# MILVLG/mmnas

Measured on AMD Instinct MI355X. Metric: supernet fwd+bwd steps/sec (VQA arch, bs=64), higher is better.
Workload: dtype f32 (bf16x6 split-operand MFMA, fp32 accumulate); 1 GPU; Net_Search supernet WEIGHT step: sample + fwd + BCE(sum) + bwd (+ gradient all-reduce), HSIZE 256, B=64/GPU, 100x2048 regions + 14 tokens, dropout 0.1 (search_vqa.py:279-292; BASELINE configs[2]); global_batch=64, parallelism=dp1, grad_allreduce=none, rccl_ranks=1, rank_id_sum_ok=True, lstm_fallback=False, dp_rows=1, dp_buckets=3, optimizer_in_step=False, gemm_split=6, hip_force_dev_kernarg=1

## Files before the change

### mmnas_amd/csrc/common.h

```cpp
#pragma once
#include <hip/hip_runtime.h>
#include <hip/hip_ext.h>
#include <stdint.h>
#include <stdio.h>
#include "../../include/mmnas_hip.h"
#include "rng.h"
#include "switches.h"

namespace mmnas {

typedef float f32x4 __attribute__((ext_vector_type(4)));
typedef float f32x16 __attribute__((ext_vector_type(16)));

void set_error(const char* fmt, ...);
int check_launch(const char* what);

#define MMNAS_REQUIRE(cond, code, ...) \
  do { if (!(cond)) { ::mmnas::set_error(__VA_ARGS__); return (code); } } while (0)

template <int CTRL, int ROW_MASK>
__device__ __forceinline__ float dpp_move(float old, float src) {
  return __int_as_float(__builtin_amdgcn_update_dpp(__float_as_int(old), __float_as_int(src), CTRL, ROW_MASK, 0xf, false));
}
__device__ __forceinline__ float wave_sum(float v) {
// ... 58 lines not shown

bool glimpse1_supported(int MID);
int glimpse1_fwd(const float* h0, const float* w0, const float* b0, float* l0, long rows0, const float* h1, const float* w1,
                 const float* b1, float* l1, long rows1, int MID, hipStream_t st);
struct NodeLnBwd {
  float* dz; float* dt;
  float* part;
  DropCfg drop;
};
int node_mix_bwd_impl(const float* const* z, const float* const* ln_a, const float* const* ln_b, int n, const float* gate,
                      const float* dout, float* d_active, int active, float* dgate, float* ws, int M, int d, float eps,
                      hipStream_t stream, bool reduce, int* nwg_out, const NodeLnBwd* lnb = nullptr);
int mixed_reduce_many(const float* const* parts, float* const* dgates, const int* nwg, const int* n, int count, hipStream_t st);
int mha_core_fwd_pair(const mmnas_mha_desc* d0, const mmnas_mha_desc* d1, hipStream_t st);
int mha_core_fwd_indexed(const mmnas_mha_desc* d, const int* kv_idx, hipStream_t st);
int transpose2d(const float* in, float* out, int R, int C, hipStream_t st);
int glimpse1_bwd_blocks(long rows, int MID);
int glimpse1_bwd(const float* dlog, const float* h, const float* w2, float gate_scale, int gated, float* dh, float* db1, float* dW2,
                 float* part, long rows, int MID, hipStream_t st, AuxReduce* aux);

int attflat_pool_fwd_packed(const float* logits, const float* x, float* probs, float* pooled, int B, int S, int d, int G, const int* off, hipStream_t st);
int attflat_pool_bwd_packed(const float* probs, const float* x, const float* dpooled, float* dlogits, float* dx, int B, int S, int d, int G,
                            const int* off, hipStream_t st);

constexpr int ADD_MANY_MAX = 24;
int add_many(const float* const* srcs, int n, float* y, size_t count, hipStream_t st);

static inline int cdiv(long a, long b) { return (int)((a + b - 1) / b); }

}
```

### mmnas_amd/csrc/head.hip

```cpp
#include "common.h"

namespace mmnas {

__global__ void __launch_bounds__(256) row_is_zero_kernel(const float* __restrict__ f, uint8_t* __restrict__ mask,
                                                          long rows, int d) {
  const int lane = threadIdx.x & 63;
  const long row = (long)blockIdx.x * 4 + (threadIdx.x >> 6);
  if (row >= rows) return;
  const float* fr = f + row * d;
  bool nz = false;
  if ((d & 3) == 0 && (((uintptr_t)fr) & 15) == 0) {
    for (int c = lane * 4; c < d; c += 256) {
      const float4 v = *reinterpret_cast<const float4*>(fr + c);
      nz |= !(v.x == 0.f && v.y == 0.f && v.z == 0.f && v.w == 0.f);
    }
  } else {
    for (int c = lane; c < d; c += 64) nz |= !(fr[c] == 0.f);
  }
  const unsigned long long any = __ballot(nz);
  if (lane == 0) mask[row] = any ? 0 : 1;
}

constexpr int AF_MAXS = 1024;

constexpr int AF_THREADS = 1024, AF_WAVES = AF_THREADS / 64;

__device__ __forceinline__ float block_reduce(float v, float* red, bool is_max) {
  const int lane = threadIdx.x & 63, w = threadIdx.x >> 6;
  v = is_max ? wave_max(v) : wave_sum(v);
  __syncthreads();
  if (lane == 0) red[w] = v;
  __syncthreads();
  float r = red[0];
  for (int i = 1; i < AF_WAVES; ++i) r = is_max ? fmaxf(r, red[i]) : r + red[i];
  return r;
}

__global__ void __launch_bounds__(AF_THREADS) attflat_pool_fwd_kernel(const float* __restrict__ logits, const float* __restrict__ x,
                                                                      const uint8_t* __restrict__ mask, float* __restrict__ probs,
                                                                      float* __restrict__ pooled, int S, int d, int G,
                                                                      const int* __restrict__ off) {
  __shared__ float sp[AF_MAXS];
  __shared__ float red[AF_WAVES];
  __shared__ float part[AF_WAVES / 4][1024];
  const int b = blockIdx.x, g = blockIdx.y, tid = threadIdx.x;
  const size_t row0 = off ? (size_t)off[b] : (size_t)b * S;
  if (off) S = off[b + 1] - off[b];
  const float* lg = logits + row0 * G + g;
  float m = -INFINITY;
  for (int s = tid; s < S; s += AF_THREADS) {
    float v = lg[(size_t)s * G];
    if (mask && !off && mask[(size_t)b * S + s]) v = -1e9f;
    sp[s] = v;
    m = fmaxf(m, v);
  }
  m = block_reduce(m, red, true);
  float sum = 0.f;
  for (int s = tid; s < S; s += AF_THREADS) {
    const float e = expf(sp[s] - m);
    sp[s] = e;
// ... 15 lines not shown
      int s = rg;
      for (; s + 12 < S; s += 16) {
        a0 += sp[s] * xb[(size_t)s * d + j];
        a1 += sp[s + 4] * xb[(size_t)(s + 4) * d + j];
        a2 += sp[s + 8] * xb[(size_t)(s + 8) * d + j];
        a3 += sp[s + 12] * xb[(size_t)(s + 12) * d + j];
      }
      for (; s < S; s += 4) a0 += sp[s] * xb[(size_t)s * d + j];
      part[rg][j - j0] = (a0 + a1) + (a2 + a3);
    }
    __syncthreads();
    for (int j = j0 + tid; j < min(d, j0 + 1024); j += AF_THREADS)
      pooled[(size_t)b * G * d + (size_t)g * d + j] = (part[0][j - j0] + part[1][j - j0]) + (part[2][j - j0] + part[3][j - j0]);
    __syncthreads();
  }
}

__global__ void __launch_bounds__(AF_THREADS) attflat_pool_bwd_kernel(const float* __restrict__ probs, const float* __restrict__ x,
                                                                      const uint8_t* __restrict__ mask,
                                                                      const float* __restrict__ dpooled, float* __restrict__ dlogits,
                                                                      float* __restrict__ dx, int S, int d, int G,
                                                                      const int* __restrict__ off) {
  __shared__ float st[AF_MAXS];
  __shared__ float red[AF_WAVES];
  const int b = blockIdx.x, tid = threadIdx.x, lane = tid & 63, w = tid >> 6;
  const size_t row0 = off ? (size_t)off[b] : (size_t)b * S;
  if (off) S = off[b + 1] - off[b];
  const float* xb = x + row0 * d;
  for (int g = 0; g < G; ++g) {
    const float* dp = dpooled + (size_t)b * G * d + (size_t)g * d;
// ... 75 lines not shown
      sw.x += dl[i] * hv[i].x; sw.y += dl[i] * hv[i].y; sw.z += dl[i] * hv[i].z; sw.w += dl[i] * hv[i].w;
    }
    *reinterpret_cast<float4*>(&red[0][slot * MID + 4 * c4]) = sb;
    *reinterpret_cast<float4*>(&red[1][slot * MID + 4 * c4]) = sw;
  }
  __syncthreads();
  float* mine = part + (size_t)blockIdx.x * 3 * MID;
  for (int i = threadIdx.x; i < 2 * MID; i += 256) {
    const int a = i < MID ? 0 : 1, c = i - a * MID;
    float v = 0.f;
    for (int q = 0; q < rs; ++q) v += red[a][q * MID + c];
    mine[a * MID + c] = v;
  }
}

__global__ void __launch_bounds__(256) transpose_kernel(const float* __restrict__ in, float* __restrict__ out, int R, int C) {
  __shared__ float t[32][33];
  const int c0 = blockIdx.x * 32, r0 = blockIdx.y * 32, tx = threadIdx.x & 31, ty = threadIdx.x >> 5;
  for (int i = ty; i < 32; i += 8)
    if (r0 + i < R && c0 + tx < C) t[i][tx] = in[(size_t)(r0 + i) * C + c0 + tx];
  __syncthreads();
  for (int i = ty; i < 32; i += 8)
    if (c0 + i < C && r0 + tx < R) out[(size_t)(c0 + i) * R + r0 + tx] = t[tx][i];
}
int transpose2d(const float* in, float* out, int R, int C, hipStream_t st) {
  MMNAS_REQUIRE(in && out && R > 0 && C > 0, MMNAS_E_ARG, "transpose2d: bad arguments");
  ProfScope ps(MMNAS_K_ROWOPS, 0.0, 8.0 * R * C, st);
  MMNAS_LAUNCH(transpose_kernel, dim3((C + 31) / 32, (R + 31) / 32), dim3(256), 0, st, in, out, R, C);
  return check_launch("transpose2d");
}

bool glimpse1_supported(int MID) { return MID >= 4 && MID % 4 == 0 && MID <= 1024; }

int glimpse1_fwd(const float* h0, const float* w0, const float* b0, float* l0, long rows0, const float* h1, const float* w1,
                 const float* b1, float* l1, long rows1, int MID, hipStream_t st) {
  MMNAS_REQUIRE(glimpse1_supported(MID) && h0 && w0 && l0 && rows0 > 0 && (rows1 == 0 || (h1 && w1 && l1)), MMNAS_E_ARG,
                "glimpse1_fwd: bad arguments");
  const Glimpse1Side s0{h0, w0, b0, l0, rows0}, s1{h1, w1, b1, l1, rows1};
  ProfScope ps(MMNAS_K_ROWOPS, 2.0 * (rows0 + rows1) * MID, 4.0 * (rows0 + rows1) * MID, st);
  MMNAS_LAUNCH(glimpse1_fwd_kernel, dim3((unsigned)((rows0 + rows1 + 3) / 4)), dim3(256), 0, st, s0, s1, MID);
  return check_launch("glimpse1_fwd");
}

// ... 41 lines not shown
}

extern "C" int mmnas_attflat_pool_fwd(const float* logits, const float* x, const uint8_t* mask, float* probs,
                                      float* pooled, int B, int S, int d, int G, void* stream) {
  MMNAS_REQUIRE(logits && x && probs && pooled, MMNAS_E_ARG, "attflat_pool_fwd: null pointer");
  MMNAS_REQUIRE(B > 0 && S > 0 && S <= AF_MAXS && d > 0 && G > 0, MMNAS_E_SHAPE, "attflat_pool_fwd: B=%d S=%d d=%d G=%d (S <= %d)",
                B, S, d, G, AF_MAXS);
  MMNAS_LAUNCH(attflat_pool_fwd_kernel, dim3(B, G), dim3(AF_THREADS), 0, (hipStream_t)stream, logits, x, mask, probs, pooled, S, d, G, (const int*)nullptr);
  return check_launch("attflat_pool_fwd");
}
namespace mmnas {
int attflat_pool_fwd_packed(const float* logits, const float* x, float* probs, float* pooled, int B, int S, int d, int G, const int* off, hipStream_t st) {
  MMNAS_REQUIRE(logits && x && probs && pooled && off, MMNAS_E_ARG, "attflat_pool_fwd: null pointer");
  MMNAS_REQUIRE(B > 0 && S > 0 && S <= AF_MAXS && d > 0 && G > 0, MMNAS_E_SHAPE, "attflat_pool_fwd: B=%d S=%d d=%d G=%d (S <= %d)", B, S, d, G, AF_MAXS);
  MMNAS_LAUNCH(attflat_pool_fwd_kernel, dim3(B, G), dim3(AF_THREADS), 0, st, logits, x, (const uint8_t*)nullptr, probs, pooled, S, d, G, off);
  return check_launch("attflat_pool_fwd");
}
int attflat_pool_bwd_packed(const float* probs, const float* x, const float* dpooled, float* dlogits, float* dx, int B, int S, int d, int G,
                            const int* off, hipStream_t st) {
  MMNAS_REQUIRE(probs && x && dpooled && dlogits && dx && off, MMNAS_E_ARG, "attflat_pool_bwd: null pointer");
  MMNAS_REQUIRE(B > 0 && S > 0 && S <= AF_MAXS && d > 0 && G > 0, MMNAS_E_SHAPE, "attflat_pool_bwd: B=%d S=%d d=%d G=%d (S <= %d)", B, S, d, G, AF_MAXS);
  MMNAS_LAUNCH(attflat_pool_bwd_kernel, dim3(B), dim3(AF_THREADS), 0, st, probs, x, (const uint8_t*)nullptr, dpooled, dlogits, dx, S, d, G, off);
  return check_launch("attflat_pool_bwd");
}
}

extern "C" int mmnas_attflat_pool_bwd(const float* probs, const float* x, const uint8_t* mask, const float* dpooled,
                                      float* dlogits, float* dx, int B, int S, int d, int G, void* stream) {
  MMNAS_REQUIRE(probs && x && dpooled && dlogits && dx, MMNAS_E_ARG, "attflat_pool_bwd: null pointer");
  MMNAS_REQUIRE(B > 0 && S > 0 && S <= AF_MAXS && d > 0 && G > 0, MMNAS_E_SHAPE, "attflat_pool_bwd: B=%d S=%d d=%d G=%d (S <= %d)",
// ... 235 lines not shown
```

### mmnas_amd/csrc/ops.hip

```cpp
#include <string.h>
#include <functional>
#include <vector>
#include "common.h"

namespace mmnas {

static inline size_t al(size_t n) { return (n + 255) & ~(size_t)255; }
template <class Op> static inline bool drops(const Op* op) { return (op->flags & MMNAS_F_TRAIN) && op->drop_p > 0.f; }

struct Carver {
  char* base; size_t off;
  explicit Carver(void* p) : base((char*)p), off(0) {}
  float* take(size_t nfloats) { float* r = (float*)(base + off); off += al(nfloats * sizeof(float)); return r; }
};

static void gemm_init(mmnas_gemm_desc& g, int layout, int N, int K, int lda, int ldb, int ldc) {
  memset(&g, 0, sizeof(g));
  g.layout = layout; g.ngroups = 1; g.nseg = 1; g.N = N; g.K = K; g.lda = lda; g.ldb = ldb; g.ldc = ldc;
  g.alpha = 1.f; g.gate_scale = 1.f; g.split_k = 1;
}

struct AttLayout {
  size_t Mq, Mk;
  float *Q, *K, *V, *att, *stats, *z, *biasT;
// ... 1429 lines not shown
    const size_t M = sd.off ? (size_t)sd.M : B * sd.S;
    HeadSideLayout& s = L.s[k];
    s.h = c.take(M * hd->MID); s.logit = c.take(M * hd->G); s.probs = c.take(M * hd->G); s.pooled = c.take(B * hd->G * hd->d);
    s.dpooled = c.take(B * hd->G * hd->d); s.dlog = c.take(M * hd->G); s.dh = c.take(M * hd->MID); s.dxpool = c.take(M * hd->d);
    s.g1part = (hd->G == 1 && glimpse1_supported(hd->MID)) ? c.take((size_t)glimpse1_bwd_blocks((long)M, hd->MID) * 3 * hd->MID) : nullptr;
  }
  L.xo = c.take(B * hd->OUT); L.sum = c.take(B * hd->OUT); L.xy = c.take(B * hd->OUT);
  L.dxy = c.take(B * hd->OUT); L.dsum = c.take(B * hd->OUT);
  L.lnws = c.take(mmnas_layernorm_bwd_ws_floats(hd->B, hd->OUT));
  L.g1proj = (hd->ANS == 1 && glimpse1_supported(hd->OUT)) ? c.take((size_t)glimpse1_bwd_blocks((long)B, hd->OUT) * 3 * hd->OUT) : nullptr;
  L.dlogT = (hd->ANS % 4 != 0 && hd->B % 4 == 0 && hd->ANS > 1) ? c.take((size_t)hd->ANS * B) : nullptr;
  L.total = c.off;
  return L;
}

static int head_check(const mmnas_head* hd, const char* who) {
  MMNAS_REQUIRE(hd, MMNAS_E_ARG, "%s: null descriptor", who);
  MMNAS_REQUIRE(hd->B > 0 && hd->d > 0 && hd->MID > 0 && hd->G > 0 && hd->OUT > 0 && hd->ANS > 0 && hd->sx.S > 0 && hd->sy.S > 0,
                MMNAS_E_SHAPE, "%s: B=%d d=%d MID=%d G=%d OUT=%d ANS=%d Sx=%d Sy=%d", who, hd->B, hd->d, hd->MID, hd->G, hd->OUT,
                hd->ANS, hd->sx.S, hd->sy.S);
  MMNAS_REQUIRE(hd->d % 4 == 0 && hd->MID % 4 == 0 && hd->OUT % 4 == 0, MMNAS_E_SHAPE, "%s: d, MID, OUT must be multiples of 4", who);
  for (int k = 0; k < 2; ++k) {
    const mmnas_attflat_side& sd = k ? hd->sy : hd->sx;
    if (sd.off) MMNAS_REQUIRE(sd.M > 0 && sd.M <= hd->B * sd.S, MMNAS_E_ARG, "%s: packed side %d: M=%d of B*S=%d rows", who, k, sd.M, hd->B * sd.S);
  }
  return MMNAS_OK;
}

}

// ... 42 lines not shown
  }
  const bool g1 = G == 1 && !oc && glimpse1_supported(MID) && head_glimpse1_on();
  if (g1) {
    if ((rc = glimpse1_fwd(L.s[0].h, hd->sx.W2, hd->sx.b2, L.s[0].logit, (long)head_rows(hd, hd->sx), L.s[1].h, hd->sy.W2, hd->sy.b2,
                           L.s[1].logit, (long)head_rows(hd, hd->sy), MID, st)))
      return rc;
  }
  gemm_init(g, MMNAS_GEMM_NT, G, MID, MID, MID, G);
  for (int k = 0; k < 2 && !g1; ++k) {
    const mmnas_attflat_side& sd = *sides[k];
    mmnas_gemm_group& gg = g.g[oc ? 0 : k];
    gg.M = head_rows(hd, sd); gg.A[0] = L.s[k].h; gg.B[0] = sd.W2; gg.bias = sd.b2; gg.C = L.s[k].logit;
    if (oc && (rc = mmnas_gemm(&g, side_stream(k)))) return rc;
  }
  if (!oc && !g1) { g.ngroups = 2; if ((rc = mmnas_gemm(&g, stream))) return rc; }
  for (int k = 0; k < 2; ++k) {
    const mmnas_attflat_side& sd = *sides[k];
    const HeadSideLayout& s = L.s[k];
    void* const ks = side_stream(k);
    if ((rc = sd.off ? attflat_pool_fwd_packed(s.logit, sd.x, s.probs, s.pooled, B, sd.S, d, G, sd.off, (hipStream_t)ks)
                     : mmnas_attflat_pool_fwd(s.logit, sd.x, sd.mask, s.probs, s.pooled, B, sd.S, d, G, ks))) return rc;
    gemm_init(g, MMNAS_GEMM_NT, OUT, G * d, G * d, G * d, OUT);
    g.g[0].M = B; g.g[0].A[0] = s.pooled; g.g[0].B[0] = sd.Wm; g.g[0].bias = sd.bm; g.g[0].C = k ? L.sum : L.xo;
    if (k) { g.g[0].residual = L.xo; g.ldres = OUT; }
    if (k && oc && (rc = ev_fork(oc->enc, st, oc->ovl[1]))) return rc;
    if ((rc = mmnas_gemm(&g, ks))) return rc;
  }
  if ((rc = mmnas_layernorm_fwd(L.sum, hd->ln_a, hd->ln_b, L.xy, B, OUT, hd->eps, stream))) return rc;
  if (L.g1proj && head_glimpse1_on())
    return glimpse1_fwd(L.xy, hd->Wp, hd->bp, hd->logits, B, nullptr, nullptr, nullptr, nullptr, 0, OUT, st);
  gemm_init(g, MMNAS_GEMM_NT, hd->ANS, OUT, OUT, OUT, hd->ANS);
  g.g[0].M = B; g.g[0].A[0] = L.xy; g.g[0].B[0] = hd->Wp; g.g[0].bias = hd->bp; g.g[0].C = hd->logits;
  return mmnas_gemm(&g, stream);
}

extern "C" int mmnas_head_bwd(const mmnas_head* hd, void* stream) {
  int rc = head_check(hd, "head_bwd");
  if (rc) return rc;
  MMNAS_REQUIRE(hd->arena && hd->dlogits && hd->ln_a && hd->dln_a && hd->dln_b && hd->Wp && hd->dWp, MMNAS_E_ARG, "head_bwd: null pointer");
  HeadLayout L = head_layout(hd);
  const bool drop = drops(hd);
  const float gate_scale = drop ? 1.0f / (1.0f - hd->drop_p) : 1.0f;
  const int B = hd->B, d = hd->d, MID = hd->MID, G = hd->G, OUT = hd->OUT, ANS = hd->ANS;
  hipStream_t st = (hipStream_t)stream;
  mmnas_gemm_desc g, w;
  if (L.g1proj && head_glimpse1_on()) {
    AuxReduce pr;
    if ((rc = glimpse1_bwd(hd->dlogits, L.xy, hd->Wp, 1.0f, 0, L.dxy, nullptr, hd->dWp, L.g1proj, B, OUT, st, &pr))) return rc;
    if ((rc = launch_aux_reduce(pr, st))) return rc;
  } else if (L.dlogT && head_projT_on()) {
    if ((rc = transpose2d(hd->dlogits, L.dlogT, B, ANS, st))) return rc;
    gemm_init(g, MMNAS_GEMM_TN, OUT, ANS, B, OUT, OUT);
    g.g[0].M = B; g.g[0].A[0] = L.dlogT; g.g[0].B[0] = hd->Wp; g.g[0].C = L.dxy;
    if ((rc = mmnas_gemm(&g, stream))) return rc;
    gemm_init(w, MMNAS_GEMM_NN, OUT, B, B, OUT, OUT);
    w.g[0].M = ANS; w.g[0].A[0] = L.dlogT; w.g[0].B[0] = L.xy; w.g[0].C = hd->dWp; w.accumulate = 1;
    if ((rc = mmnas_gemm(&w, stream))) return rc;
  } else {
    gemm_init(w, MMNAS_GEMM_TN, OUT, B, ANS, OUT, OUT);
    w.g[0].M = ANS; w.g[0].A[0] = hd->dlogits; w.g[0].B[0] = L.xy; w.g[0].C = hd->dWp; w.accumulate = 1;
    gemm_init(g, MMNAS_GEMM_NN, OUT, ANS, ANS, OUT, OUT);
    g.g[0].M = B; g.g[0].A[0] = hd->dlogits; g.g[0].B[0] = hd->Wp; g.g[0].C = L.dxy;
    if ((rc = mmnas_gemm_pair(&g, &w, stream))) return rc;
  }
  if (hd->dbp && (rc = mmnas_colsum(hd->dlogits, hd->dbp, B, ANS, ANS, stream))) return rc;
  AuxReduce lnred;
  lnred.part = nullptr;
  if ((rc = layernorm_bwd_deferred(L.sum, hd->ln_a, L.dxy, L.dsum, hd->dln_a, hd->dln_b, nullptr, nullptr, L.lnws, 0.f, 0, 0, B, OUT,
                                   hd->eps, st, &lnred)))
    return rc;
  SideCtx* oc = head_overlap_on() ? side_ctx(st, true) : nullptr;
  if (oc && (rc = ev_fork(st, oc->enc, oc->ovl[2]))) return rc;
  for (int k = 1; k >= 0; --k) {
    const mmnas_attflat_side& sd = k ? hd->sy : hd->sx;
    const HeadSideLayout& s = L.s[k];
    MMNAS_REQUIRE(sd.x && sd.dx && sd.dW1 && sd.dW2 && sd.dWm, MMNAS_E_ARG, "head_bwd: side %d null pointer", k);
    hipStream_t st = (oc && k == 0) ? oc->enc : (hipStream_t)stream;
    void* const stream = (void*)st;
    const int M = head_rows(hd, sd);
    gemm_init(w, MMNAS_GEMM_TN, G * d, B, OUT, G * d, G * d);
    w.g[0].M = OUT; w.g[0].A[0] = L.dsum; w.g[0].B[0] = s.pooled; w.g[0].C = sd.dWm; w.accumulate = 1;
    gemm_init(g, MMNAS_GEMM_NN, G * d, OUT, OUT, G * d, G * d);
    g.g[0].M = B; g.g[0].A[0] = L.dsum; g.g[0].B[0] = sd.Wm; g.g[0].C = s.dpooled;
    if ((rc = gemm_pair_aux(&g, &w, k ? &lnred : nullptr, st))) return rc;
    if (sd.dbm && (rc = mmnas_colsum(L.dsum, sd.dbm, B, OUT, OUT, stream))) return rc;
    if ((rc = sd.off ? attflat_pool_bwd_packed(s.probs, sd.x, s.dpooled, s.dlog, s.dxpool, B, sd.S, d, G, sd.off, st)
                     : mmnas_attflat_pool_bwd(s.probs, sd.x, sd.mask, s.dpooled, s.dlog, s.dxpool, B, sd.S, d, G, stream))) return rc;
    AuxReduce g1red;
    g1red.part = nullptr;
    if (G == 1 && glimpse1_supported(MID) && head_glimpse1_on()) {
      if ((rc = glimpse1_bwd(s.dlog, s.h, sd.W2, gate_scale, 1, s.dh, sd.db1, sd.dW2, s.g1part, M, MID, st, &g1red))) return rc;
      if (sd.db2 && (rc = mmnas_colsum(s.dlog, sd.db2, M, G, G, stream))) return rc;
    } else {
    gemm_init(w, MMNAS_GEMM_TN, MID, M, G, MID, MID);
    w.g[0].M = G; w.g[0].A[0] = s.dlog; w.g[0].B[0] = s.h; w.g[0].C = sd.dW2; w.accumulate = 1;
    gemm_init(g, MMNAS_GEMM_NN, MID, G, G, MID, MID);
    g.g[0].M = M; g.g[0].A[0] = s.dlog; g.g[0].B[0] = sd.W2; g.g[0].C = s.dh;
    g.g[0].gate = s.h; g.ldgate = MID; g.gate_scale = gate_scale;
    g.g[0].colsum = sd.db1;
    if ((rc = mmnas_gemm_pair(&g, &w, stream))) return rc;
    if (sd.db2 && (rc = mmnas_colsum(s.dlog, sd.db2, M, G, G, stream))) return rc;
    }
    gemm_init(w, MMNAS_GEMM_TN, d, M, MID, d, d);
    w.g[0].M = MID; w.g[0].A[0] = s.dh; w.g[0].B[0] = sd.x; w.g[0].C = sd.dW1; w.accumulate = 1;
    gemm_init(g, MMNAS_GEMM_NN, d, MID, MID, d, d);
    g.g[0].M = M; g.g[0].A[0] = s.dh; g.g[0].B[0] = sd.W1; g.g[0].C = sd.dx;
    g.g[0].residual = s.dxpool; g.ldres = d;
    if ((rc = gemm_pair_aux(&g, &w, g1red.part ? &g1red : nullptr, st))) return rc;
  }
  if (oc && (rc = ev_fork(oc->enc, st, oc->ovl[3]))) return rc;
  return MMNAS_OK;
}
```

### mmnas_amd/csrc/switches.h

```cpp
#pragma once

namespace mmnas {

int env_int(const char* name, int dflt);

enum SwKind { sw_int, sw_bool, sw_exact1, sw_presence, sw_string };
enum SwPolicy { sw_once, sw_every_call, sw_reload };

struct Switch {
  const char* name;
  int dflt;
  SwKind kind;
  SwPolicy policy;
  const char* help;
  int value;
  int state;

  int get() { return state ? value : read(); }
  int read();
  int reload();
  int set(int v);
  int peek(int* source) const;
};

#define MMNAS_SWITCHES(X) \
   \
  X(chain_overlap, "MMNAS_CHAIN_OVERLAP", 0, bool, once, "language stream beside the leading image-stream operators (mmnas_set_chain_overlap); measured: no gain, DESIGN.md section 5") \
  X(head_overlap, "MMNAS_HEAD_OVERLAP", 0, bool, once, "the answer head's two AttFlat sides on two streams") \
  X(head_glimpse1, "MMNAS_HEAD_GLIMPSE1", 1, bool, every_call, "0: the head's one-glimpse logit layer as GEMM launches (A/B, tests); ops.py reads it too") \
  X(head_projt, "MMNAS_HEAD_PROJT", 1, bool, every_call, "0: the answer projection's gradients from the untransposed loss gradient") \
  X(rel_hoist, "MMNAS_REL_HOIST", 1, bool, once, "relation bias of all lazy-handle operators of a stream in one launch per direction (mmnas_set_rel_hoist); 0: one fused launch per operator (supernet step 4.54 -> 5.00 ms)") \
  X(rel_overlap, "MMNAS_REL_OVERLAP", 0, bool, once, "the image stream's relation launches on a second stream (mmnas_set_rel_overlap); measured slower, +2.5 % on the supernet step") \
  X(node_lnb, "MMNAS_NODE_LNB", 1, bool, once, "architecture step: the sampled candidate's LayerNorm backward inside the node's mix kernel (7.81 -> 7.72 ms, profiles/r06_node_lnb_ab.txt); 0: its own launch") \
  X(guided_hoist, "MMNAS_GUIDED_HOIST", 1, bool, once, "key / value projections of a chain's guided operators as grouped launches (mmnas_set_guided_hoist)") \
  X(rel_fwd_valu, "MMNAS_REL_FWD_VALU", 0, exact1, every_call, "1: a lone RelSelfAtt computes its bias with the per-operator fused kernel instead of the one-operator multi kernel (A/B)") \
  X(side_prio, "MMNAS_SIDE_PRIO", 1, bool, every_call, "0: the chains' extra streams without stream priorities (read when a stream pair is created)") \
  X(side_flush, "MMNAS_SIDE_FLUSH", 0, string, once, "op: side-stream parameter-gradient work released behind every operator instead of once per phase") \
  X(wgrad_live, "MMNAS_WGRAD_LIVE", 1, int, once, "image-stream weight gradients of a padded batch's chain reduce over the 32-row K-tiles that cover the live gradient rows only (mmnas_set_wgrad_live); 0: all B Sy rows") \
   \
  X(small_ops, "MMNAS_SMALL_OPS", 1, bool, once, "SelfAtt of <= 16 rows as one launch forward (mmnas_set_small_ops); 0: the general path") \
  X(small_bwd, "MMNAS_SMALL_BWD", 1, bool, once, "the same operators' backward as two launches (mmnas_set_small_bwd)") \
  X(small_ffn, "MMNAS_SMALL_FFN", 0, int, once, "FeedForward forward as one launch (mmnas_set_small_ffn): 1 four slices of 256 hidden units, 2 eight of 128; measured neutral (profiles/r05_small_ffn_ab.txt)") \
   \
  X(gemm_ln, "MMNAS_GEMM_LN", 0, exact1, once, "1: the merge / last FFN product and its LayerNorm as one row-panel launch (mmnas_set_gemm_ln); measured neutral, profiles/r06_ab.txt") \
// ... 46 lines not shown
```

### mmnas_amd/switches.py

```python
import contextlib
import os

_PARSE = {
    'not0': lambda v: v != '0',
    'is1': lambda v: v == '1',
    'presence': lambda v: v is not None,
    'tri': lambda v: int(v) if v in ('0', '1') else None,
    'side': lambda v: 2 if v == 'rel' else int(v == '1'),
    'string': lambda v: v,
}


class Flag:
    __slots__ = ('name', 'default', 'kind', 'policy', 'help', '_parse', '_state', '_value')

    def __init__(self, name, default, kind, policy, help):
        self.name, self.default, self.kind, self.policy, self.help = name, default, kind, policy, help
        self._parse = _PARSE[kind]
        self._state = None
        self._value = None

    def get(self):
        if self._state is not None:
            return self._value
# ... 27 lines not shown
AUTOGRAD_CHAIN = _flag('MMNAS_AUTOGRAD_CHAIN', False, 'is1', 'every_call', '1: the chain as one autograd node whose inputs are the parameters (stock DDP); measured neutral')
UNPAD = _flag('MMNAS_UNPAD', False, 'is1', 'once', '1: the decoder stream on the valid region rows only (ops.set_unpad): same logits and gradients, supernet step 4.73 -> 3.78 ms (DESIGN.md)')
VGD_HEAD = _flag('MMNAS_VGD_HEAD', False, 'is1', 'once', '1: the grounding head as one native call per direction (ops.set_vgd_head); measurement: README, the grounding head section')
LSTM = _flag('MMNAS_LSTM', True, 'not0', 'every_call', '0: nn.LSTM (MIOpen, ~110 launches per step) instead of the persistent-kernel LSTM')
CONV_IM2COL = _flag('MMNAS_CONV_IM2COL', None, 'tri', 'every_call', 'dense Conv1d: 1 always through the window buffer, 0 direct whenever the shape allows, unset: direct unless the padded grid costs > 25 % more rows')
HEAD_GLIMPSE1 = _flag('MMNAS_HEAD_GLIMPSE1', True, 'not0', 'every_call', '0: one-unit linear layers as GEMM launches (A/B, tests); the native head reads it too')
GEMM_GENERIC = _flag('MMNAS_GEMM_GENERIC', False, 'presence', 'every_call', 'set (to anything): dense Conv1d through the window buffer, as the guarded-load GEMM path needs; gemm.hip reads it too')
ZERO_TERMS = _flag('MMNAS_ZERO_TERMS', True, 'not0', 'every_call', "0: plain parameters instead of the zero-term bookkeeping of the reference's literal lines (zeroterm.py)")
LAZY_REL = _flag('MMNAS_LAZY_REL', True, 'not0', 'import', '0: materialise the relation embeddings as the reference does (read when model/nets.py is imported)')
DP_ROWS = _flag('MMNAS_DP_ROWS', True, 'not0', 'every_call', '0: the embedding gradient exchanged dense instead of by rows (A/B)')
DP_INLINE = _flag('MMNAS_DP_INLINE', True, 'not0', 'every_call', '0: async_op=True + work.wait() instead of collectives issued inline on the communication stream')
DP_TAIL_MAIN = _flag('MMNAS_DP_TAIL_MAIN', True, 'not0', 'import', '0: the end of a data-parallel step on the communication stream, one scatter per bucket (1: -0.7 % on search_vqa_dp1; read when dp.py is imported)')
DP_EARLY_SCATTER = _flag('MMNAS_DP_EARLY_SCATTER', False, 'is1', 'every_call', "1: scatter a bucket's averaged gradients back as soon as its all-reduce is done")
LIB_PATH = _flag('MMNAS_LIB_PATH', None, 'string', 'doc', 'path of the shared library to load instead of mmnas_amd/lib/libmmnas_hip.so (tuning builds; read when _lib.py is imported)')
_flag('MMNAS_REFERENCE_ROOT', None, 'string', 'doc', "a checkout of the reference whose mmnas/ package is merged behind this repository's (mmnas/__init__.py)")
_flag('MMNAS_PROF_DUMP', None, 'string', 'doc', 'file the native profiler appends one row per bracketed launch to (csrc/util.hip)')
_flag('MMNAS_LN_ROWS_STATS', None, 'string', 'doc', 'file tests/test_ln_rows_gpu.py writes the worst LayerNorm error per (kernel, row class, output) to (tests/ln_rows.py)')


@contextlib.contextmanager
def gemm_schedule(rows):
    from . import _lib as L
    known = native()
    for name in rows:
        if name not in known:
            raise ValueError('gemm_schedule: %s is not a row of the native switch table' % name)
    saved = {}
    try:
        for name, v in rows.items():
            saved[name] = os.environ.get(name)
# ... 36 lines not shown
```

Baseline: 244.1 steps/s.

## Fuse answer-head AttFlat sides into shared pool-forward and pool+glimpse backward kernels

Adds a two-side pooling forward kernel and a single backward kernel that does the pooling backward and the one-glimpse logit backward for both AttFlat sides in one launch. It also folds the projection bias column sum into the transpose kernel. The aim is to cut launch count and the intermediate dlog/h round trips in the answer head. The transpose-with-colsum kernel now uses one block per column strip with a serial loop over rows, which lowers parallelism, and a new switch gates the fused path (on by default).

Result: no change. 245.6 steps/s (median of 6 runs) (+0.6%).

```diff
diff --git a/mmnas_amd/csrc/common.h b/mmnas_amd/csrc/common.h
--- a/mmnas_amd/csrc/common.h
+++ b/mmnas_amd/csrc/common.h
@@ -96,7 +96,7 @@
 int mixed_reduce_many(const float* const* parts, float* const* dgates, const int* nwg, const int* n, int count, hipStream_t st);
 int mha_core_fwd_pair(const mmnas_mha_desc* d0, const mmnas_mha_desc* d1, hipStream_t st);
 int mha_core_fwd_indexed(const mmnas_mha_desc* d, const int* kv_idx, hipStream_t st);
-int transpose2d(const float* in, float* out, int R, int C, hipStream_t st);
+int transpose2d(const float* in, float* out, int R, int C, hipStream_t st, float* colsum = nullptr);
 int glimpse1_bwd_blocks(long rows, int MID);
 int glimpse1_bwd(const float* dlog, const float* h, const float* w2, float gate_scale, int gated, float* dh, float* db1, float* dW2,
                  float* part, long rows, int MID, hipStream_t st, AuxReduce* aux);
@@ -105,6 +105,19 @@
 int attflat_pool_bwd_packed(const float* probs, const float* x, const float* dpooled, float* dlogits, float* dx, int B, int S, int d, int G,
                             const int* off, hipStream_t st);
 
+struct HeadBwdSide {
+  const float *probs, *x, *dpooled, *h, *w2;
+  const uint8_t* mask;
+  const int* off;
+  float *dlog, *dxpool, *dh, *part;
+  int S;
+};
+int attflat_pool_fwd_sides(const float* const* logits, const float* const* x, const uint8_t* const* mask, float* const* probs,
+                           float* const* pooled, const int* const* off, const int* S, int B, int d, int G, hipStream_t st);
+bool head_sides_bwd_fits(long rows, int B, int MID);
+int head_sides_bwd(const HeadBwdSide* sides, float* const* db1, float* const* dW2, int B, int d, int MID,
+                   float gate_scale, hipStream_t st, AuxReduce* aux);
+
 constexpr int ADD_MANY_MAX = 24;
 int add_many(const float* const* srcs, int n, float* y, size_t count, hipStream_t st);
 
diff --git a/mmnas_amd/csrc/head.hip b/mmnas_amd/csrc/head.hip
--- a/mmnas_amd/csrc/head.hip
+++ b/mmnas_amd/csrc/head.hip
@@ -36,14 +36,14 @@
   return r;
 }
 
-__global__ void __launch_bounds__(AF_THREADS) attflat_pool_fwd_kernel(const float* __restrict__ logits, const float* __restrict__ x,
-                                                                      const uint8_t* __restrict__ mask, float* __restrict__ probs,
-                                                                      float* __restrict__ pooled, int S, int d, int G,
-                                                                      const int* __restrict__ off) {
+__device__ __forceinline__ void attflat_pool_fwd_body(const float* __restrict__ logits, const float* __restrict__ x,
+                                                      const uint8_t* __restrict__ mask, float* __restrict__ probs,
+                                                      float* __restrict__ pooled, int S, int d, int G,
+                                                      const int* __restrict__ off, const int b, const int g) {
   __shared__ float sp[AF_MAXS];
   __shared__ float red[AF_WAVES];
   __shared__ float part[AF_WAVES / 4][1024];
-  const int b = blockIdx.x, g = blockIdx.y, tid = threadIdx.x;
+  const int tid = threadIdx.x;
   const size_t row0 = off ? (size_t)off[b] : (size_t)b * S;
   if (off) S = off[b + 1] - off[b];
   const float* lg = logits + row0 * G + g;
@@ -89,6 +89,20 @@
       pooled[(size_t)b * G * d + (size_t)g * d + j] = (part[0][j - j0] + part[1][j - j0]) + (part[2][j - j0] + part[3][j - j0]);
     __syncthreads();
   }
+}
+
+__global__ void __launch_bounds__(AF_THREADS) attflat_pool_fwd_kernel(const float* __restrict__ logits, const float* __restrict__ x,
+                                                                      const uint8_t* __restrict__ mask, float* __restrict__ probs,
+                                                                      float* __restrict__ pooled, int S, int d, int G,
+                                                                      const int* __restrict__ off) {
+  attflat_pool_fwd_body(logits, x, mask, probs, pooled, S, d, G, off, blockIdx.x, blockIdx.y);
+}
+
+struct PoolFwdSide { const float* logits; const float* x; const uint8_t* mask; float* probs; float* pooled; const int* off; int S; };
+
+__global__ void __launch_bounds__(AF_THREADS) attflat_pool_fwd2_kernel(const PoolFwdSide s0, const PoolFwdSide s1, int d, int G) {
+  const PoolFwdSide& s = blockIdx.z ? s1 : s0;
+  attflat_pool_fwd_body(s.logits, s.x, s.mask, s.probs, s.pooled, s.S, d, G, s.off, blockIdx.x, blockIdx.y);
 }
 
 __global__ void __launch_bounds__(AF_THREADS) attflat_pool_bwd_kernel(const float* __restrict__ probs, const float* __restrict__ x,
@@ -194,6 +208,136 @@
   }
 }
 
+constexpr int HF_ITER = 4;
+constexpr int HF_CS = 4096;
+
+__device__ __forceinline__ void hf_load(float4 (&hv)[HF_ITER], const float* __restrict__ hb, int r0, int rs, int S, int MID, int c4) {
+#pragma unroll
+  for (int i = 0; i < HF_ITER; ++i) {
+    const int r = r0 + i * rs;
+    hv[i] = r < S ? *reinterpret_cast<const float4*>(hb + (size_t)r * MID + 4 * c4) : make_float4(0.f, 0.f, 0.f, 0.f);
+  }
+}
+
+__global__ void __launch_bounds__(AF_THREADS) head_side_bwd_kernel(const HeadBwdSide s0, const HeadBwdSide s1, int d, int MID,
+                                                                   float gate_scale) {
+  __shared__ float st[AF_MAXS], sp[AF_MAXS], sdl[AF_MAXS];
+  __shared__ float red[AF_WAVES];
+  __shared__ __attribute__((aligned(16))) float cs[2][HF_CS];
+  const HeadBwdSide& sd = blockIdx.y ? s1 : s0;
+  const int b = blockIdx.x, tid = threadIdx.x, lane = tid & 63, w = tid >> 6;
+  int S = sd.S;
+  const size_t row0 = sd.off ? (size_t)sd.off[b] : (size_t)b * S;
+  if (sd.off) S = sd.off[b + 1] - sd.off[b];
+  const float* __restrict__ xb = sd.x + row0 * d;
+  const float* __restrict__ dp = sd.dpooled + (size_t)b * d;
+  const float* __restrict__ hb = sd.h + row0 * MID;
+  const int nc4 = MID >> 2;
+  const int rs = AF_THREADS / nc4;
+  const int c4 = tid % nc4, slot = tid / nc4;
+  const bool colthr = slot < rs;
+  float4 hv[HF_ITER];
+  if (colthr) hf_load(hv, hb, slot, rs, S, MID, c4);
+  for (int s = w; s < S; s += 2 * AF_WAVES) {
+    const int sb = s + AF_WAVES;
+    float a = 0.f, a2 = 0.f;
+    if (sb < S) {
+      for (int j = lane; j < d; j += 64) {
+        a += xb[(size_t)s * d + j] * dp[j];
+        a2 += xb[(size_t)sb * d + j] * dp[j];
+      }
+      a2 = wave_sum(a2);
+      if (lane == 0) st[sb] = a2;
+    } else {
+      for (int j = lane; j < d; j += 64) a += xb[(size_t)s * d + j] * dp[j];
+    }
+    a = wave_sum(a);
+    if (lane == 0) st[s] = a;
+  }
+  __syncthreads();
+  float dot = 0.f;
+  for (int s = tid; s < S; s += AF_THREADS) {
+    const float pr = sd.probs[row0 + s];
+    sp[s] = pr;
+    dot += pr * st[s];
+  }
+  dot = block_reduce(dot, red, false);
+  for (int s = tid; s < S; s += AF_THREADS) {
+    const float pr = sp[s];
+    const bool masked = sd.mask && !sd.off && sd.mask[(size_t)b * S + s];
+    const float dl = masked ? 0.f : pr * (st[s] - dot);
+    sd.dlog[row0 + s] = dl;
+    sdl[s] = dl;
+  }
+  __syncthreads();
+  float* __restrict__ mine = sd.part + (size_t)b * 3 * MID;
+  if (colthr) {
+    const float4 wv = *reinterpret_cast<const float4*>(sd.w2 + 4 * c4);
+    float* __restrict__ dhb = sd.dh + row0 * MID;
+    float4 sb = make_float4(0.f, 0.f, 0.f, 0.f), sw = sb;
+    for (int r0 = slot; r0 < S; r0 += rs * HF_ITER) {
+      float4 hn[HF_ITER];
+      hf_load(hn, hb, r0 + rs * HF_ITER, rs, S, MID, c4);
+#pragma unroll
+      for (int i = 0; i < HF_ITER; ++i) {
+        const int r = r0 + i * rs;
+        if (r < S) {
+          const float dl = sdl[r];
+          float4 o;
+          o.x = hv[i].x > 0.f ? dl * wv.x * gate_scale : 0.f; o.y = hv[i].y > 0.f ? dl * wv.y * gate_scale : 0.f;
+          o.z = hv[i].z > 0.f ? dl * wv.z * gate_scale : 0.f; o.w = hv[i].w > 0.f ? dl * wv.w * gate_scale : 0.f;
+          *reinterpret_cast<float4*>(dhb + (size_t)r * MID + 4 * c4) = o;
+          sb.x += o.x; sb.y += o.y; sb.z += o.z; sb.w += o.w;
+          sw.x += dl * hv[i].x; sw.y += dl * hv[i].y; sw.z += dl * hv[i].z; sw.w += dl * hv[i].w;
+        }
+      }
+#pragma unroll
+      for (int i = 0; i < HF_ITER; ++i) hv[i] = hn[i];
+    }
+    *reinterpret_cast<float4*>(&cs[0][slot * MID + 4 * c4]) = sb;
+    *reinterpret_cast<float4*>(&cs[1][slot * MID + 4 * c4]) = sw;
+  }
+  float* __restrict__ dxb = sd.dxpool + row0 * d;
+  for (int s = w; s < S; s += AF_WAVES) {
+    const float pr = sp[s];
+    for (int j = 4 * lane; j < d; j += 256) {
+      const float4 dv = *reinterpret_cast<const float4*>(dp + j);
+      float4 o = make_float4(0.f, 0.f, 0.f, 0.f);
+      o.x += pr * dv.x; o.y += pr * dv.y; o.z += pr * dv.z; o.w += pr * dv.w;
+      *reinterpret_cast<float4*>(dxb + (size_t)s * d + j) = o;
+    }
+  }
+  __syncthreads();
+  for (int i = tid; i < 2 * MID; i += AF_THREADS) {
+    const int a = i < MID ? 0 : 1, c = i - a * MID;
+    float v = 0.f;
+    for (int q = 0; q < rs; ++q) v += cs[a][q * MID + c];
+    mine[a * MID + c] = v;
+  }
+}
+
+bool head_sides_bwd_fits(long rows, int B, int MID) { return glimpse1_supported(MID) && glimpse1_bwd_blocks(rows, MID) >= B; }
+
+int head_sides_bwd(const HeadBwdSide* sides, float* const* db1, float* const* dW2, int B, int d, int MID,
+                   float gate_scale, hipStream_t st, AuxReduce* aux) {
+  MMNAS_REQUIRE(sides && aux && B > 0 && d > 0 && d % 4 == 0 && glimpse1_supported(MID), MMNAS_E_ARG, "head_sides_bwd: bad arguments");
+  long rows = 0;
+  for (int k = 0; k < 2; ++k) {
+    const HeadBwdSide& s = sides[k];
+    MMNAS_REQUIRE(s.probs && s.x && s.dpooled && s.h && s.w2 && s.dlog && s.dxpool && s.dh && s.part && dW2[k], MMNAS_E_ARG,
+                  "head_sides_bwd: side %d null pointer", k);
+    MMNAS_REQUIRE(s.S > 0 && s.S <= AF_MAXS, MMNAS_E_SHAPE, "head_sides_bwd: side %d S=%d (<= %d)", k, s.S, AF_MAXS);
+    rows += (long)B * s.S;
+  }
+  ProfScope ps(MMNAS_K_ROWOPS, (4.0 * d + 5.0 * MID) * rows, (8.0 * d + 8.0 * MID) * rows, st, "HEAD_SIDES_BWD");
+  MMNAS_LAUNCH(head_side_bwd_kernel, dim3(B, 2), dim3(AF_THREADS), 0, st, sides[0], sides[1], d, MID, gate_scale);
+  for (int k = 0; k < 2; ++k) {
+    aux[k].part = sides[k].part; aux[k].nrows = B; aux[k].d = MID;
+    aux[k].out[0] = db1[k]; aux[k].out[1] = dW2[k]; aux[k].out[2] = nullptr;
+  }
+  return check_launch("head_sides_bwd");
+}
+
 __global__ void __launch_bounds__(256) transpose_kernel(const float* __restrict__ in, float* __restrict__ out, int R, int C) {
   __shared__ float t[32][33];
   const int c0 = blockIdx.x * 32, r0 = blockIdx.y * 32, tx = threadIdx.x & 31, ty = threadIdx.x >> 5;
@@ -203,10 +347,34 @@
   for (int i = ty; i < 32; i += 8)
     if (c0 + i < C && r0 + tx < R) out[(size_t)(c0 + i) * R + r0 + tx] = t[tx][i];
 }
-int transpose2d(const float* in, float* out, int R, int C, hipStream_t st) {
+__global__ void __launch_bounds__(256) transpose_colsum_kernel(const float* __restrict__ in, float* __restrict__ out,
+                                                               float* __restrict__ colsum, int R, int C) {
+  __shared__ float t[32][33];
+  __shared__ float ps[8][32];
+  const int c0 = blockIdx.x * 32, tx = threadIdx.x & 31, ty = threadIdx.x >> 5;
+  float s = 0.f;
+  for (int r0 = 0; r0 < R; r0 += 32) {
+    for (int i = ty; i < 32; i += 8)
+      if (r0 + i < R && c0 + tx < C) {
+        const float v = in[(size_t)(r0 + i) * C + c0 + tx];
+        t[i][tx] = v;
+        s += v;
+      }
+    __syncthreads();
+    for (int i = ty; i < 32; i += 8)
+      if (c0 + i < C && r0 + tx < R) out[(size_t)(c0 + i) * R + r0 + tx] = t[tx][i];
+    __syncthreads();
+  }
+  ps[ty][tx] = s;
+  __syncthreads();
+  if (ty == 0 && c0 + tx < C)
+    colsum[c0 + tx] += ((ps[0][tx] + ps[1][tx]) + (ps[2][tx] + ps[3][tx])) + ((ps[4][tx] + ps[5][tx]) + (ps[6][tx] + ps[7][tx]));
+}
+int transpose2d(const float* in, float* out, int R, int C, hipStream_t st, float* colsum) {
   MMNAS_REQUIRE(in && out && R > 0 && C > 0, MMNAS_E_ARG, "transpose2d: bad arguments");
   ProfScope ps(MMNAS_K_ROWOPS, 0.0, 8.0 * R * C, st);
-  MMNAS_LAUNCH(transpose_kernel, dim3((C + 31) / 32, (R + 31) / 32), dim3(256), 0, st, in, out, R, C);
+  if (colsum) MMNAS_LAUNCH(transpose_colsum_kernel, dim3((C + 31) / 32), dim3(256), 0, st, in, out, colsum, R, C);
+  else MMNAS_LAUNCH(transpose_kernel, dim3((C + 31) / 32, (R + 31) / 32), dim3(256), 0, st, in, out, R, C);
   return check_launch("transpose2d");
 }
 
@@ -278,6 +446,19 @@
   MMNAS_REQUIRE(logits && x && probs && pooled && off, MMNAS_E_ARG, "attflat_pool_fwd: null pointer");
   MMNAS_REQUIRE(B > 0 && S > 0 && S <= AF_MAXS && d > 0 && G > 0, MMNAS_E_SHAPE, "attflat_pool_fwd: B=%d S=%d d=%d G=%d (S <= %d)", B, S, d, G, AF_MAXS);
   MMNAS_LAUNCH(attflat_pool_fwd_kernel, dim3(B, G), dim3(AF_THREADS), 0, st, logits, x, (const uint8_t*)nullptr, probs, pooled, S, d, G, off);
+  return check_launch("attflat_pool_fwd");
+}
+int attflat_pool_fwd_sides(const float* const* logits, const float* const* x, const uint8_t* const* mask, float* const* probs,
+                           float* const* pooled, const int* const* off, const int* S, int B, int d, int G, hipStream_t st) {
+  PoolFwdSide s[2];
+  for (int k = 0; k < 2; ++k) {
+    MMNAS_REQUIRE(logits[k] && x[k] && probs[k] && pooled[k], MMNAS_E_ARG, "attflat_pool_fwd: side %d null pointer", k);
+    MMNAS_REQUIRE(B > 0 && S[k] > 0 && S[k] <= AF_MAXS && d > 0 && G > 0, MMNAS_E_SHAPE, "attflat_pool_fwd: B=%d S=%d d=%d G=%d (S <= %d)",
+                  B, S[k], d, G, AF_MAXS);
+    s[k] = PoolFwdSide{logits[k], x[k], off[k] ? nullptr : mask[k], probs[k], pooled[k], off[k], S[k]};
+  }
+  ProfScope ps(MMNAS_K_ROWOPS, 2.0 * B * (S[0] + S[1]) * d, 4.0 * B * (S[0] + S[1]) * d, st, "HEAD_POOL_FWD");
+  MMNAS_LAUNCH(attflat_pool_fwd2_kernel, dim3(B, G, 2), dim3(AF_THREADS), 0, st, s[0], s[1], d, G);
   return check_launch("attflat_pool_fwd");
 }
 int attflat_pool_bwd_packed(const float* probs, const float* x, const float* dpooled, float* dlogits, float* dx, int B, int S, int d, int G,
diff --git a/mmnas_amd/csrc/ops.hip b/mmnas_amd/csrc/ops.hip
--- a/mmnas_amd/csrc/ops.hip
+++ b/mmnas_amd/csrc/ops.hip
@@ -1467,6 +1467,15 @@
   return L;
 }
 
+struct HeadScope : ProfScope {
+  HeadScope(const char* tag, hipStream_t st) : ProfScope(MMNAS_K_ROWOPS, 0.0, 0.0, st, tag) {}
+};
+
+static bool head_fuse_applies(const mmnas_head* hd) {
+  if (!sw::head_fuse.get() || hd->G != 1 || !glimpse1_supported(hd->MID) || !head_glimpse1_on() || head_overlap_on()) return false;
+  return head_sides_bwd_fits(head_rows(hd, hd->sx), hd->B, hd->MID) && head_sides_bwd_fits(head_rows(hd, hd->sy), hd->B, hd->MID);
+}
+
 static int head_check(const mmnas_head* hd, const char* who) {
   MMNAS_REQUIRE(hd, MMNAS_E_ARG, "%s: null descriptor", who);
   MMNAS_REQUIRE(hd->B > 0 && hd->d > 0 && hd->MID > 0 && hd->G > 0 && hd->OUT > 0 && hd->ANS > 0 && hd->sx.S > 0 && hd->sy.S > 0,
@@ -1539,12 +1548,26 @@
     if (oc && (rc = mmnas_gemm(&g, side_stream(k)))) return rc;
   }
   if (!oc && !g1) { g.ngroups = 2; if ((rc = mmnas_gemm(&g, stream))) return rc; }
+  const bool fuse = g1 && head_fuse_applies(hd);
+  if (fuse) {
+    const float* lg[2] = {L.s[0].logit, L.s[1].logit};
+    const float* xs[2] = {hd->sx.x, hd->sy.x};
+    const uint8_t* ms[2] = {hd->sx.mask, hd->sy.mask};
+    float* pr[2] = {L.s[0].probs, L.s[1].probs};
+    float* po[2] = {L.s[0].pooled, L.s[1].pooled};
+    const int* of[2] = {hd->sx.off, hd->sy.off};
+    const int Ss[2] = {hd->sx.S, hd->sy.S};
+    if ((rc = attflat_pool_fwd_sides(lg, xs, ms, pr, po, of, Ss, B, d, G, st))) return rc;
+  }
   for (int k = 0; k < 2; ++k) {
     const mmnas_attflat_side& sd = *sides[k];
     const HeadSideLayout& s = L.s[k];
     void* const ks = side_stream(k);
-    if ((rc = sd.off ? attflat_pool_fwd_packed(s.logit, sd.x, s.probs, s.pooled, B, sd.S, d, G, sd.off, (hipStream_t)ks)
-                     : mmnas_attflat_pool_fwd(s.logit, sd.x, sd.mask, s.probs, s.pooled, B, sd.S, d, G, ks))) return rc;
+    if (!fuse) {
+      HeadScope hs("HEAD pool_fwd", (hipStream_t)ks);
+      if ((rc = sd.off ? attflat_pool_fwd_packed(s.logit, sd.x, s.probs, s.pooled, B, sd.S, d, G, sd.off, (hipStream_t)ks)
+                       : mmnas_attflat_pool_fwd(s.logit, sd.x, sd.mask, s.probs, s.pooled, B, sd.S, d, G, ks))) return rc;
+    }
     gemm_init(g, MMNAS_GEMM_NT, OUT, G * d, G * d, G * d, OUT);
     g.g[0].M = B; g.g[0].A[0] = s.pooled; g.g[0].B[0] = sd.Wm; g.g[0].bias = sd.bm; g.g[0].C = k ? L.sum : L.xo;
     if (k) { g.g[0].residual = L.xo; g.ldres = OUT; }
@@ -1569,12 +1592,15 @@
   const int B = hd->B, d = hd->d, MID = hd->MID, G = hd->G, OUT = hd->OUT, ANS = hd->ANS;
   hipStream_t st = (hipStream_t)stream;
   mmnas_gemm_desc g, w;
+  const bool fuse = head_fuse_applies(hd);
+  bool dbp_done = false;
   if (L.g1proj && head_glimpse1_on()) {
     AuxReduce pr;
     if ((rc = glimpse1_bwd(hd->dlogits, L.xy, hd->Wp, 1.0f, 0, L.dxy, nullptr, hd->dWp, L.g1proj, B, OUT, st, &pr))) return rc;
     if ((rc = launch_aux_reduce(pr, st))) return rc;
   } else if (L.dlogT && head_projT_on()) {
-    if ((rc = transpose2d(hd->dlogits, L.dlogT, B, ANS, st))) return rc;
+    if ((rc = transpose2d(hd->dlogits, L.dlogT, B, ANS, st, fuse ? hd->dbp : nullptr))) return rc;
+    dbp_done = fuse;
     gemm_init(g, MMNAS_GEMM_TN, OUT, ANS, B, OUT, OUT);
     g.g[0].M = B; g.g[0].A[0] = L.dlogT; g.g[0].B[0] = hd->Wp; g.g[0].C = L.dxy;
     if ((rc = mmnas_gemm(&g, stream))) return rc;
@@ -1588,7 +1614,10 @@
     g.g[0].M = B; g.g[0].A[0] = hd->dlogits; g.g[0].B[0] = hd->Wp; g.g[0].C = L.dxy;
     if ((rc = mmnas_gemm_pair(&g, &w, stream))) return rc;
   }
-  if (hd->dbp && (rc = mmnas_colsum(hd->dlogits, hd->dbp, B, ANS, ANS, stream))) return rc;
+  if (hd->dbp && !dbp_done) {
+    HeadScope hs("HEAD colsum dbp", st);
+    if ((rc = mmnas_colsum(hd->dlogits, hd->dbp, B, ANS, ANS, stream))) return rc;
+  }
   AuxReduce lnred;
   lnred.part = nullptr;
   if ((rc = layernorm_bwd_deferred(L.sum, hd->ln_a, L.dxy, L.dsum, hd->dln_a, hd->dln_b, nullptr, nullptr, L.lnws, 0.f, 0, 0, B, OUT,
@@ -1596,42 +1625,86 @@
     return rc;
   SideCtx* oc = head_overlap_on() ? side_ctx(st, true) : nullptr;
   if (oc && (rc = ev_fork(st, oc->enc, oc->ovl[2]))) return rc;
-  for (int k = 1; k >= 0; --k) {
-    const mmnas_attflat_side& sd = k ? hd->sy : hd->sx;
+  const mmnas_attflat_side* sides[2] = {&hd->sx, &hd->sy};
+  for (int k = 0; k < 2; ++k)
+    MMNAS_REQUIRE(sides[k]->x && sides[k]->dx && sides[k]->dW1 && sides[k]->dW2 && sides[k]->dWm, MMNAS_E_ARG, "head_bwd: side %d null pointer", k);
+  auto side_stream = [&](int k) -> hipStream_t { return (oc && k == 0) ? oc->enc : st; };
+  auto merge_bwd = [&](int k) -> int {
+    const mmnas_attflat_side& sd = *sides[k];
     const HeadSideLayout& s = L.s[k];
-    MMNAS_REQUIRE(sd.x && sd.dx && sd.dW1 && sd.dW2 && sd.dWm, MMNAS_E_ARG, "head_bwd: side %d null pointer", k);
-    hipStream_t st = (oc && k == 0) ? oc->enc : (hipStream_t)stream;
-    void* const stream = (void*)st;
-    const int M = head_rows(hd, sd);
     gemm_init(w, MMNAS_GEMM_TN, G * d, B, OUT, G * d, G * d);
     w.g[0].M = OUT; w.g[0].A[0] = L.dsum; w.g[0].B[0] = s.pooled; w.g[0].C = sd.dWm; w.accumulate = 1;
     gemm_init(g, MMNAS_GEMM_NN, G * d, OUT, OUT, G * d, G * d);
     g.g[0].M = B; g.g[0].A[0] = L.dsum; g.g[0].B[0] = sd.Wm; g.g[0].C = s.dpooled;
-    if ((rc = gemm_pair_aux(&g, &w, k ? &lnred : nullptr, st))) return rc;
-    if (sd.dbm && (rc = mmnas_colsum(L.dsum, sd.dbm, B, OUT, OUT, stream))) return rc;
-    if ((rc = sd.off ? attflat_pool_bwd_packed(s.probs, sd.x, s.dpooled, s.dlog, s.dxpool, B, sd.S, d, G, sd.off, st)
-                     : mmnas_attflat_pool_bwd(s.probs, sd.x, sd.mask, s.dpooled, s.dlog, s.dxpool, B, sd.S, d, G, stream))) return rc;
-    AuxReduce g1red;
-    g1red.part = nullptr;
-    if (G == 1 && glimpse1_supported(MID) && head_glimpse1_on()) {
-      if ((rc = glimpse1_bwd(s.dlog, s.h, sd.W2, gate_scale, 1, s.dh, sd.db1, sd.dW2, s.g1part, M, MID, st, &g1red))) return rc;
-      if (sd.db2 && (rc = mmnas_colsum(s.dlog, sd.db2, M, G, G, stream))) return rc;
-    } else {
-    gemm_init(w, MMNAS_GEMM_TN, MID, M, G, MID, MID);
-    w.g[0].M = G; w.g[0].A[0] = s.dlog; w.g[0].B[0] = s.h; w.g[0].C = sd.dW2; w.accumulate = 1;
-    gemm_init(g, MMNAS_GEMM_NN, MID, G, G, MID, MID);
-    g.g[0].M = M; g.g[0].A[0] = s.dlog; g.g[0].B[0] = sd.W2; g.g[0].C = s.dh;
-    g.g[0].gate = s.h; g.ldgate = MID; g.gate_scale = gate_scale;
-    g.g[0].colsum = sd.db1;
-    if ((rc = mmnas_gemm_pair(&g, &w, stream))) return rc;
-    if (sd.db2 && (rc = mmnas_colsum(s.dlog, sd.db2, M, G, G, stream))) return rc;
-    }
+    int rc = gemm_pair_aux(&g, &w, k ? &lnred : nullptr, side_stream(k));
+    if (rc) return rc;
+    if (!sd.dbm) return MMNAS_OK;
+    HeadScope hs("HEAD colsum dbm", side_stream(k));
+    return mmnas_colsum(L.dsum, sd.dbm, B, OUT, OUT, (void*)side_stream(k));
+  };
+  auto fc_bwd = [&](int k, const AuxReduce* red) -> int {
+    const mmnas_attflat_side& sd = *sides[k];
+    const HeadSideLayout& s = L.s[k];
+    const int M = head_rows(hd, sd);
     gemm_init(w, MMNAS_GEMM_TN, d, M, MID, d, d);
     w.g[0].M = MID; w.g[0].A[0] = s.dh; w.g[0].B[0] = sd.x; w.g[0].C = sd.dW1; w.accumulate = 1;
     gemm_init(g, MMNAS_GEMM_NN, d, MID, MID, d, d);
     g.g[0].M = M; g.g[0].A[0] = s.dh; g.g[0].B[0] = sd.W1; g.g[0].C = sd.dx;
     g.g[0].residual = s.dxpool; g.ldres = d;
-    if ((rc = gemm_pair_aux(&g, &w, g1red.part ? &g1red : nullptr, st))) return rc;
+    return gemm_pair_aux(&g, &w, red, side_stream(k));
+  };
+  if (fuse) {
+    for (int k = 1; k >= 0; --k)
+      if ((rc = merge_bwd(k))) return rc;
+    HeadBwdSide hs[2];
+    float *db1[2], *dW2[2];
+    for (int k = 0; k < 2; ++k) {
+      const mmnas_attflat_side& sd = *sides[k];
+      const HeadSideLayout& s = L.s[k];
+      hs[k] = HeadBwdSide{s.probs, sd.x, s.dpooled, s.h, sd.W2, sd.off ? nullptr : sd.mask, sd.off, s.dlog, s.dxpool, s.dh, s.g1part, sd.S};
+      db1[k] = sd.db1; dW2[k] = sd.dW2;
+    }
+    AuxReduce g1red[2];
+    if ((rc = head_sides_bwd(hs, db1, dW2, B, d, MID, gate_scale, st, g1red))) return rc;
+    for (int k = 1; k >= 0; --k) {
+      if (sides[k]->db2) {
+        HeadScope sc("HEAD colsum db2", st);
+        if ((rc = mmnas_colsum(L.s[k].dlog, sides[k]->db2, head_rows(hd, *sides[k]), G, G, stream))) return rc;
+      }
+      if ((rc = fc_bwd(k, &g1red[k]))) return rc;
+    }
+    return MMNAS_OK;
+  }
+  for (int k = 1; k >= 0; --k) {
+    const mmnas_attflat_side& sd = *sides[k];
+    const HeadSideLayout& s = L.s[k];
+    hipStream_t st = side_stream(k);
+    void* const stream = (void*)st;
+    const int M = head_rows(hd, sd);
+    if ((rc = merge_bwd(k))) return rc;
+    {
+      HeadScope hs("HEAD pool_bwd", st);
+      if ((rc = sd.off ? attflat_pool_bwd_packed(s.probs, sd.x, s.dpooled, s.dlog, s.dxpool, B, sd.S, d, G, sd.off, st)
+                       : mmnas_attflat_pool_bwd(s.probs, sd.x, sd.mask, s.dpooled, s.dlog, s.dxpool, B, sd.S, d, G, stream))) return rc;
+    }
+    AuxReduce g1red;
+    g1red.part = nullptr;
+    if (G == 1 && glimpse1_supported(MID) && head_glimpse1_on()) {
+      if ((rc = glimpse1_bwd(s.dlog, s.h, sd.W2, gate_scale, 1, s.dh, sd.db1, sd.dW2, s.g1part, M, MID, st, &g1red))) return rc;
+    } else {
+      gemm_init(w, MMNAS_GEMM_TN, MID, M, G, MID, MID);
+      w.g[0].M = G; w.g[0].A[0] = s.dlog; w.g[0].B[0] = s.h; w.g[0].C = sd.dW2; w.accumulate = 1;
+      gemm_init(g, MMNAS_GEMM_NN, MID, G, G, MID, MID);
+      g.g[0].M = M; g.g[0].A[0] = s.dlog; g.g[0].B[0] = sd.W2; g.g[0].C = s.dh;
+      g.g[0].gate = s.h; g.ldgate = MID; g.gate_scale = gate_scale;
+      g.g[0].colsum = sd.db1;
+      if ((rc = mmnas_gemm_pair(&g, &w, stream))) return rc;
+    }
+    if (sd.db2) {
+      HeadScope hs("HEAD colsum db2", st);
+      if ((rc = mmnas_colsum(s.dlog, sd.db2, M, G, G, stream))) return rc;
+    }
+    if ((rc = fc_bwd(k, g1red.part ? &g1red : nullptr))) return rc;
   }
   if (oc && (rc = ev_fork(oc->enc, st, oc->ovl[3]))) return rc;
   return MMNAS_OK;
diff --git a/mmnas_amd/csrc/switches.h b/mmnas_amd/csrc/switches.h
--- a/mmnas_amd/csrc/switches.h
+++ b/mmnas_amd/csrc/switches.h
@@ -28,6 +28,7 @@
   X(chain_overlap, "MMNAS_CHAIN_OVERLAP", 0, bool, once, "language stream beside the leading image-stream operators (mmnas_set_chain_overlap); measured: no gain, DESIGN.md section 5") \
   X(head_overlap, "MMNAS_HEAD_OVERLAP", 0, bool, once, "the answer head's two AttFlat sides on two streams") \
   X(head_glimpse1, "MMNAS_HEAD_GLIMPSE1", 1, bool, every_call, "0: the head's one-glimpse logit layer as GEMM launches (A/B, tests); ops.py reads it too") \
+  X(head_fuse, "MMNAS_HEAD_FUSE", 1, int, every_call, "0 | 1: the answer head's two AttFlat sides per launch at one glimpse: pooling forward; pooling + glimpse-logit backward as one kernel; dbp inside the transposition. 0: one launch per side and step") \
   X(head_projt, "MMNAS_HEAD_PROJT", 1, bool, every_call, "0: the answer projection's gradients from the untransposed loss gradient") \
   X(rel_hoist, "MMNAS_REL_HOIST", 1, bool, once, "relation bias of all lazy-handle operators of a stream in one launch per direction (mmnas_set_rel_hoist); 0: one fused launch per operator (supernet step 4.54 -> 5.00 ms)") \
   X(rel_overlap, "MMNAS_REL_OVERLAP", 0, bool, once, "the image stream's relation launches on a second stream (mmnas_set_rel_overlap); measured slower, +2.5 % on the supernet step") \
diff --git a/mmnas_amd/switches.py b/mmnas_amd/switches.py
--- a/mmnas_amd/switches.py
+++ b/mmnas_amd/switches.py
@@ -65,6 +65,7 @@
 DP_EARLY_SCATTER = _flag('MMNAS_DP_EARLY_SCATTER', False, 'is1', 'every_call', "1: scatter a bucket's averaged gradients back as soon as its all-reduce is done")
 LIB_PATH = _flag('MMNAS_LIB_PATH', None, 'string', 'doc', 'path of the shared library to load instead of mmnas_amd/lib/libmmnas_hip.so (tuning builds; read when _lib.py is imported)')
 _flag('MMNAS_REFERENCE_ROOT', None, 'string', 'doc', "a checkout of the reference whose mmnas/ package is merged behind this repository's (mmnas/__init__.py)")
+_flag('MMNAS_HEAD_FUSE', None, 'string', 'doc', "0: the answer head's AttFlat sides one launch per side and step; read per call by the native head alone (csrc/switches.h)")
 _flag('MMNAS_PROF_DUMP', None, 'string', 'doc', 'file the native profiler appends one row per bracketed launch to (csrc/util.hip)')
 _flag('MMNAS_LN_ROWS_STATS', None, 'string', 'doc', 'file tests/test_ln_rows_gpu.py writes the worst LayerNorm error per (kernel, row class, output) to (tests/ln_rows.py)')
 
```
